# saiprasadbarke/robustmvd

Measured on AMD Instinct MI355X. Metric: depth-maps/sec at 768x1152x4srcx256planes; warp+aggregate HBM GB/s vs roofline, higher is better.
Workload: dtype f32; 1 GPU; mvsnet (Path B) forward 768x1152, 4 source views, 256 planes, batch 1 per step (BASELINE.json configs[2]); the regulariser's two layers with 32 input channels (conv0, conv4): every fp32 operand as two range-scaled fp16 terms on fp16 MFMA, fp32 accumulation (at least as close to a float64 convolution as the fp32 matrix instruction over 1e-42..1e30: tests/test_hip_f16.py), the other nine layers and ; parallelism=1 independent replica(s), frames round-robin, no collectives

## Files before the change

robustmvd_amd/csrc/deconv3d_split.hip:

```cpp
#include "mvd_common.h"
#include "split_operand.h"
#include <stdlib.h>

#ifndef DS_TWO_PHASE
#define DS_TWO_PHASE 0
#endif

namespace mvd {

typedef _Float16 dsh8 __attribute__((ext_vector_type(8)));
typedef float dsf4 __attribute__((ext_vector_type(4)));
typedef unsigned int dsu4 __attribute__((ext_vector_type(4)));

constexpr int DS_TH = 4, DS_ROWS = DS_TH + 1;

template <int CIN, int MT>
struct DSGeom {
    static constexpr bool PAIR = CIN == 16;
    static constexpr int TW = 16 * MT, COLS = TW + 1;
    static constexpr int NG = CIN / 8;
    static constexpr int KS = PAIR ? 1 : CIN / 32;
    static constexpr int PIX = 2 * DS_ROWS * COLS;
    static constexpr int GS = (PIX * 16 + 255) / 256 * 256;
    static constexpr int TERM = NG * GS;
    static constexpr int LDS = 2 * TERM;
    static constexpr int ITEMS = PIX * NG, NIT = (ITEMS + 255) / 256;
    static constexpr int NCLS = PAIR ? 4 : 8;
};
static constexpr int ds_nfrag(int cin) { return cin == 16 ? 9 : 27 * (cin / 32); }
static constexpr size_t DS_FRAG_BYTES = 2 * 64 * 16;

__global__ void deconv_split_pack_kernel(const float* __restrict__ w, const float* __restrict__ eun, _Float16* __restrict__ packed, int Cin,
                                         int Cout, int nfrag, long long total) {
    const long long e = (long long)blockIdx.x * 256 + threadIdx.x;
    if (e >= total) return;
    const int j = (int)(e & 7), lane = (int)((e >> 3) & 63), term = (int)((e >> 9) & 1);
    const int f = (int)((e >> 10) % nfrag), nt = (int)((e >> 10) / nfrag);
    const int row = lane & 15, k = 8 * (lane >> 4) + j;
    int cout, cin, tap;
    if (Cin == 16) {
        const int pw = row >> 3, s = k >> 4;
        const int kw = s == 0 ? (pw ? 2 : 1) : (pw ? 0 : -1);
        cout = row & 7; cin = k & 15;
        tap = kw >= 0 ? f * 3 + kw : -1;
    } else {
        const int ks = f % (Cin / 32);
        cout = nt * 16 + row; cin = 32 * ks + k;
        tap = f / (Cin / 32);
    }
    const float v = tap >= 0 ? w[((size_t)cin * Cout + cout) * 27 + tap] / eun[nt * 16 + row] : 0.f;
    _Float16 hi, lo;
    split_weight(v, 1.0f, hi, lo);
    packed[e] = term == 0 ? hi : lo;
}

struct DSParams {
    const float* x;
    const float* xamax;
    const char* wpk;
    const float* scale;
    const float* shift;
    const float* skip;
    float* y;
    float* yamax;
    int B, Di, hi, wi, Cout, relu;
    int tiles_w, tiles_h, ncb;
};

template <int CIN, int NT, int MT, bool YAMAX>
__global__ void __launch_bounds__(256) deconv3d_split_kernel(DSParams p) {
    const float amax_seen = absmax_seen(YAMAX ? p.yamax : nullptr);
    using G = DSGeom<CIN, MT>;
    constexpr bool PAIR = G::PAIR;
    constexpr int COLS = G::COLS, NG = G::NG, KS = G::KS, GS = G::GS, TERM = G::TERM, NCLS = G::NCLS, NFRAG = ds_nfrag(CIN);
    static_assert(!PAIR || NT == 1, "the pair form has one row tile");
    extern __shared__ __attribute__((aligned(16))) char dslab[];

    const int tid = threadIdx.x;
    const int lane = tid & 63, wave = tid >> 6;
    const int vox = lane & 15, q = lane >> 4;
    int bx = blockIdx.x;
    const int cb = bx % p.ncb; bx /= p.ncb;
    const int tw = bx % p.tiles_w; bx /= p.tiles_w;
    const int th = bx % p.tiles_h; bx /= p.tiles_h;
    const int zd = bx % p.Di;
    const int b = bx / p.Di;
    const int r0 = th * DS_TH, c0 = tw * G::TW;

    float xsc, xsc_inv;
    split_xscale(p.xamax, xsc, xsc_inv);

    constexpr int NKW = PAIR ? 1 : 3;
    const char* __restrict__ wl = p.wpk + (size_t)cb * NT * NFRAG * DS_FRAG_BYTES + lane * 16;
    auto load_a = [&](int step, dsh8 (&dst)[NKW][KS][NT][2]) {
#pragma unroll
        for (int kw = 0; kw < NKW; ++kw)
#pragma unroll
            for (int ks = 0; ks < KS; ++ks)
#pragma unroll
                for (int n = 0; n < NT; ++n)
#pragma unroll
                    for (int t = 0; t < 2; ++t)
                        dst[kw][ks][n][t] = *reinterpret_cast<const dsh8*>(
                            wl + ((size_t)n * NFRAG + (step * NKW + kw) * KS + ks) * DS_FRAG_BYTES + t * 1024);
    };
    constexpr bool AHEAD = 2 * NKW * KS * NT * 2 * 4 <= 112;
    dsh8 af[NKW][KS][NT][2];
    if constexpr (AHEAD) load_a(0, af);

    float emul[NT][4], emul2[NT][4], esc[NT][4], esh[NT][4];
    {
        const float* __restrict__ eun = reinterpret_cast<const float*>(p.wpk + (size_t)p.ncb * NT * NFRAG * DS_FRAG_BYTES);
#pragma unroll
        for (int n = 0; n < NT; ++n)
#pragma unroll
            for (int k = 0; k < 4; ++k) {
                const int row = (cb * NT + n) * 16 + q * 4 + k;
                const int ch = PAIR ? (row & 7) : row;
                const int se = (int)((__float_as_uint(eun[row]) >> 23) & 0xffu) + (int)((__float_as_uint(xsc_inv) >> 23) & 0xffu) - 254;
                emul[n][k] = __uint_as_float((unsigned)(127 + (se >> 1)) << 23);
                emul2[n][k] = __uint_as_float((unsigned)(127 + se - (se >> 1)) << 23);
                esc[n][k] = p.scale[ch];
                esh[n][k] = p.shift[ch];
            }
    }

    {
        constexpr int NIT = G::NIT, C4 = CIN / 4;
        const float4* __restrict__ x4 = reinterpret_cast<const float4*>(p.x) + (size_t)b * p.Di * p.hi * p.wi * C4;
        float4 pf[NIT][2];
        bool ok[NIT];
#pragma unroll
        for (int i = 0; i < NIT; ++i) {
            const int e = tid + 256 * i;
            const int g = e % NG, pix = e / NG;
            const int col = pix % COLS, r = pix / COLS;
            const int pl = r / DS_ROWS, row = r - pl * DS_ROWS;
            const int plane = zd + pl, gr = r0 + row, gc = c0 + col;
            ok[i] = e < G::ITEMS && plane < p.Di && gr < p.hi && gc < p.wi;
            const size_t o = ok[i] ? (((size_t)plane * p.hi + gr) * p.wi + gc) * C4 + 2 * g : 0;
            pf[i][0] = x4[o];
            pf[i][1] = x4[o + 1];
        }
#pragma unroll
        for (int i = 0; i < NIT; ++i) {
            const int e = tid + 256 * i;
            const int g = e % NG, pix = e / NG;
            unsigned h[4], l[4];
            split2(xsc, pf[i][0].x, pf[i][0].y, h[0], l[0]);
            split2(xsc, pf[i][0].z, pf[i][0].w, h[1], l[1]);
            split2(xsc, pf[i][1].x, pf[i][1].y, h[2], l[2]);
            split2(xsc, pf[i][1].z, pf[i][1].w, h[3], l[3]);
            dsu4 hv = {h[0], h[1], h[2], h[3]}, lv = {l[0], l[1], l[2], l[3]};
            if (!ok[i]) { hv = dsu4{0, 0, 0, 0}; lv = dsu4{0, 0, 0, 0}; }
            if (e < G::ITEMS) {
                *reinterpret_cast<dsu4*>(dslab + g * GS + pix * 16) = hv;
                *reinterpret_cast<dsu4*>(dslab + TERM + g * GS + pix * 16) = lv;
            }
        }
    }
    __syncthreads();

    dsf4 acc[NCLS][MT][NT];
#pragma unroll
    for (int c = 0; c < NCLS; ++c)
#pragma unroll
        for (int m = 0; m < MT; ++m)
#pragma unroll
            for (int n = 0; n < NT; ++n) acc[c][m][n] = dsf4{0.f, 0.f, 0.f, 0.f};

    const char* __restrict__ lbase = dslab + (PAIR ? (q & 1) * GS + (q >> 1) * 16 : q * GS) + (wave * COLS + vox) * 16;

#pragma unroll
    for (int step = 0; step < 9; ++step) {
        const int kd = step / 3, kh = step % 3;
        dsh8 af_next[NKW][KS][NT][2];
        if constexpr (AHEAD) {
            if (step + 1 < 9) load_a(step + 1, af_next);
        } else {
            load_a(step, af);
        }
        const int rowpix = ((kd == 0 ? DS_ROWS : 0) + (kh == 0)) * COLS;
#pragma unroll
        for (int kw = 0; kw < NKW; ++kw) {
            const int cls = PAIR ? (((kd != 1) << 1) | (kh != 1)) : (((kd != 1) << 2) | ((kh != 1) << 1) | (kw != 1));
            const int colpix = PAIR ? 0 : (kw == 0);
#pragma unroll
            for (int ks = 0; ks < KS; ++ks) {
                dsh8 xh[MT], xl[MT];
#pragma unroll
                for (int m = 0; m < MT; ++m) {
                    const char* a = lbase + ks * 4 * GS + (rowpix + colpix + m * 16) * 16;
                    xh[m] = *reinterpret_cast<const dsh8*>(a);
                    xl[m] = *reinterpret_cast<const dsh8*>(a + TERM);
                }
#pragma unroll
                for (int m = 0; m < MT; ++m)
#pragma unroll
                    for (int n = 0; n < NT; ++n) {
                        acc[cls][m][n] = __builtin_amdgcn_mfma_f32_16x16x32_f16(af[kw][ks][n][0], xh[m], acc[cls][m][n], 0, 0, 0);
                        acc[cls][m][n] = __builtin_amdgcn_mfma_f32_16x16x32_f16(af[kw][ks][n][1], xh[m], acc[cls][m][n], 0, 0, 0);
                        acc[cls][m][n] = __builtin_amdgcn_mfma_f32_16x16x32_f16(af[kw][ks][n][0], xl[m], acc[cls][m][n], 0, 0, 0);
                    }
            }
        }
        if constexpr (AHEAD) {
            if (step + 1 < 9) {
#pragma unroll
                for (int kw = 0; kw < NKW; ++kw)
#pragma unroll
                    for (int ks = 0; ks < KS; ++ks)
#pragma unroll
                        for (int n = 0; n < NT; ++n) {
                            af[kw][ks][n][0] = af_next[kw][ks][n][0];
                            af[kw][ks][n][1] = af_next[kw][ks][n][1];
                        }
            }
        }
    }

    const int arow = r0 + wave;
    const bool row_ok = arow < p.hi;
    auto offset = [&](int c, int m, int n) {
        const int pd = PAIR ? c >> 1 : c >> 2, ph = PAIR ? c & 1 : (c >> 1) & 1, pw = PAIR ? q >> 1 : c & 1;
        const size_t row_base = (((size_t)b * 2 * p.Di + 2 * zd + pd) * 2 * p.hi + 2 * arow + ph) * 2 * p.wi;
        const int cbase = PAIR ? 4 * (q & 1) : (cb * NT + n) * 16 + q * 4;
        return (row_base + 2 * (c0 + m * 16 + vox) + pw) * p.Cout + cbase;
    };
    auto finish = [&](int c, int m, int n, size_t o) {
        float4 sk = make_float4(0.f, 0.f, 0.f, 0.f);
        if (p.skip) sk = *reinterpret_cast<const float4*>(p.skip + o);
        float r[4];
#pragma unroll
        for (int k = 0; k < 4; ++k) {
            float val = fmaf(acc[c][m][n][k] * emul[n][k] * emul2[n][k], esc[n][k], esh[n][k]);
            if (p.relu) val = fmaxf(val, 0.f);
            r[k] = val;
        }
        return dsf4{r[0] + sk.x, r[1] + sk.y, r[2] + sk.z, r[3] + sk.w};
    };
    if constexpr (!(YAMAX || DS_TWO_PHASE)) {
        if (row_ok) {
#pragma unroll
            for (int c = 0; c < NCLS; ++c)
#pragma unroll
                for (int m = 0; m < MT; ++m) {
                    if (c0 + m * 16 + vox >= p.wi) continue;
#pragma unroll
                    for (int n = 0; n < NT; ++n) {
                        const size_t o = offset(c, m, n);
                        *reinterpret_cast<dsf4*>(p.y + o) = finish(c, m, n, o);
                    }
                }
        }
    } else {
        [[maybe_unused]] float amax = 0.f;
        if (row_ok) {
#pragma unroll
            for (int c = 0; c < NCLS; ++c)
#pragma unroll
                for (int m = 0; m < MT; ++m) {
                    if (c0 + m * 16 + vox >= p.wi) continue;
#pragma unroll
                    for (int n = 0; n < NT; ++n) {
                        const dsf4 out = finish(c, m, n, offset(c, m, n));
                        acc[c][m][n] = out;
                        if constexpr (YAMAX)
                            amax = fmaxf(fmaxf(amax, fmaxf(finite_abs_or_zero(out[0]), finite_abs_or_zero(out[1]))),
                                         fmaxf(finite_abs_or_zero(out[2]), finite_abs_or_zero(out[3])));
                    }
                }
        }
        if constexpr (YAMAX) {
            const float m = workgroup_max(amax, reinterpret_cast<float*>(dslab + G::LDS), tid);
            if (tid == 0) {
                if (m > amax_seen) atomicMax(reinterpret_cast<unsigned*>(p.yamax), __float_as_uint(m));
            }
        }
        if (row_ok) {
#pragma unroll
            for (int c = 0; c < NCLS; ++c)
#pragma unroll
                for (int m = 0; m < MT; ++m) {
                    if (c0 + m * 16 + vox >= p.wi) continue;
#pragma unroll
                    for (int n = 0; n < NT; ++n) *reinterpret_cast<dsf4*>(p.y + offset(c, m, n)) = acc[c][m][n];
                }
        }
    }
}

template <int CIN, int NT, int MT, bool YAMAX>
static int ds_launch_v(DSParams p, hipStream_t st) {
    using G = DSGeom<CIN, MT>;
    static_assert(G::LDS <= 64 * 1024, "slab exceeds the default LDS limit");
    p.tiles_h = (p.hi + DS_TH - 1) / DS_TH;
    p.tiles_w = (p.wi + G::TW - 1) / G::TW;
    p.ncb = G::PAIR ? 1 : p.Cout / (16 * NT);
    const long long nblk = (long long)p.ncb * p.tiles_w * p.tiles_h * p.Di * p.B;
    MVD_REQUIRE(nblk <= 0x7fffffffLL, "deconv3d_split: %lld workgroups exceed the grid limit", nblk);
    hipLaunchKernelGGL((deconv3d_split_kernel<CIN, NT, MT, YAMAX>), dim3((unsigned)nblk), dim3(256), G::LDS + 16, st, p);
    return launch_status("deconv3d_split");
}
template <int CIN, int NT, int MT>
static int ds_launch(const DSParams& p, hipStream_t st) {
    return p.yamax ? ds_launch_v<CIN, NT, MT, true>(p, st) : ds_launch_v<CIN, NT, MT, false>(p, st);
}

}

static bool ds_shape_ok(int Cin, int Cout) {
    return ((Cin == 64 || Cin == 32) && Cout >= 16 && Cout <= 64 && Cout % 16 == 0) || (Cin == 16 && Cout == 8);
}
static int ds_row_tiles(int Cin, int Cout) { return Cin == 16 ? 1 : Cout / 16; }
static size_t ds_frag_bytes(int Cin, int Cout) { return (size_t)ds_row_tiles(Cin, Cout) * mvd::ds_nfrag(Cin) * mvd::DS_FRAG_BYTES; }

extern "C" {

size_t mvd_deconv3d_split_packed_weight_bytes(int Cin, int Cout) {
    return ds_shape_ok(Cin, Cout) ? ds_frag_bytes(Cin, Cout) + (size_t)ds_row_tiles(Cin, Cout) * 16 * sizeof(float) : 0;
}

int mvd_pack_deconv3d_weights_split(const float* w, int Cin, int Cout, void* packed, mvd_stream_t stream) {
    MVD_REQUIRE(w && packed, "pack_deconv3d_weights_split: NULL argument");
    MVD_REQUIRE(ds_shape_ok(Cin, Cout), "pack_deconv3d_weights_split: 32 or 64 input channels with 16, 32, 48 or 64 output channels, or 16 -> 8, are built (got %d -> %d)",
                Cin, Cout);
    float* eun = reinterpret_cast<float*>(static_cast<char*>(packed) + ds_frag_bytes(Cin, Cout));
    const int rows = ds_row_tiles(Cin, Cout) * 16;
    mvd::split_wscale_launch(w, eun, Cin, Cout, 27, true, rows, rows, (hipStream_t)stream);
    const long long total = (long long)(ds_frag_bytes(Cin, Cout) / 2);
    hipLaunchKernelGGL(mvd::deconv_split_pack_kernel, dim3((unsigned)((total + 255) / 256)), dim3(256), 0, (hipStream_t)stream, w, eun,
                       (_Float16*)packed, Cin, Cout, mvd::ds_nfrag(Cin), total);
    return mvd::launch_status("pack_deconv3d_weights_split");
}

int mvd_deconv3d_bn_relu_f32_split(const float* x, const float* x_absmax, const void* packed_w, const float* scale, const float* shift,
                                   const float* skip, float* y, float* y_absmax, int B, int Di, int hi, int wi, int Cin, int Cout, int relu,
                                   mvd_stream_t stream) {
    MVD_REQUIRE(x && x_absmax && packed_w && scale && shift && y, "deconv3d_split: NULL argument");
    MVD_REQUIRE(ds_shape_ok(Cin, Cout), "deconv3d_split: 32 or 64 input channels with 16, 32, 48 or 64 output channels, or 16 -> 8, are built (got %d -> %d)", Cin, Cout);
    MVD_REQUIRE(B > 0 && Di > 0 && hi > 0 && wi > 0, "deconv3d_split: non-positive dimension");
    mvd::DSParams p{};
    p.x = x; p.xamax = x_absmax; p.wpk = (const char*)packed_w; p.scale = scale; p.shift = shift; p.skip = skip; p.y = y; p.yamax = y_absmax;
    p.B = B; p.Di = Di; p.hi = hi; p.wi = wi; p.Cout = Cout; p.relu = relu;
    hipStream_t st = (hipStream_t)stream;
    int cfg = 0;
    if (const char* e = mvd::exp_env("MVD_DS_CFG")) cfg = atoi(e);
    if (Cin == 16) return cfg % 10 == 3 ? mvd::ds_launch<16, 1, 3>(p, st) : mvd::ds_launch<16, 1, 2>(p, st);
    if (Cin == 32) return cfg % 10 == 2 ? mvd::ds_launch<32, 1, 2>(p, st) : mvd::ds_launch<32, 1, 1>(p, st);
    if (cfg / 10 == 2 && Cout % 32 == 0) return mvd::ds_launch<64, 2, 1>(p, st);
    return mvd::ds_launch<64, 1, 1>(p, st);
}
}
```

Before: 340.7 depth-maps/sec.

## Add persistent deconv3d split kernel with prefetched slabs and rolling weight lookahead

Adds a persistent-grid variant of the split-fp16 transposed 3D convolution in which each workgroup loops over tiles. While computing the current tile it prefetches the next tile's input slab and skip values into registers and streams the per-step weight fragments LA steps ahead. For the 16-channel pair form, all weights stay resident. It is enabled by default for the 64-, 32- and 16-input-channel default configurations, and aims to hide global-memory latency and launch/tail overhead. The cost is much higher register pressure, with launch bounds limiting waves per SIMD, and a grid sized to two workgroups per CU equivalent, which may reduce occupancy.

```diff
diff --git a/robustmvd_amd/csrc/deconv3d_split.hip b/robustmvd_amd/csrc/deconv3d_split.hip
--- a/robustmvd_amd/csrc/deconv3d_split.hip
+++ b/robustmvd_amd/csrc/deconv3d_split.hip
@@ -4,6 +4,9 @@
 
 #ifndef DS_TWO_PHASE
 #define DS_TWO_PHASE 0
+#endif
+#ifndef DS_STAGE_PIXMAJOR
+#define DS_STAGE_PIXMAJOR 0
 #endif
 
 namespace mvd {
@@ -65,6 +68,7 @@
     float* yamax;
     int B, Di, hi, wi, Cout, relu;
     int tiles_w, tiles_h, ncb;
+    int tiles;
 };
 
 template <int CIN, int NT, int MT, bool YAMAX>
@@ -290,7 +294,282 @@
     }
 }
 
-template <int CIN, int NT, int MT, bool YAMAX>
+template <int CIN, int NT, int MT, bool YAMAX, int LA, int WAVES, bool SKIP_EARLY, bool PIXMAJOR>
+__global__ void __launch_bounds__(256, WAVES) deconv3d_split_persist_kernel(DSParams p) {
+    const float amax_seen = absmax_seen(YAMAX ? p.yamax : nullptr);
+    using G = DSGeom<CIN, MT>;
+    constexpr bool PAIR = G::PAIR;
+    constexpr int COLS = G::COLS, NG = G::NG, KS = G::KS, GS = G::GS, TERM = G::TERM, NCLS = G::NCLS, NFRAG = ds_nfrag(CIN);
+    constexpr int NIT = G::NIT, C4 = CIN / 4, NKW = PAIR ? 1 : 3;
+    static_assert(!PAIR || NT == 1, "the pair form has one row tile");
+    static_assert(LA >= 1 && LA <= 9 && (LA < 9 || PAIR), "resident weights: the pair form (one channel block) only");
+    static_assert(NIT <= 32, "one bit per staging item");
+    extern __shared__ __attribute__((aligned(16))) char dslab[];
+
+    const int tid = threadIdx.x;
+    const int lane = tid & 63, wave = __builtin_amdgcn_readfirstlane(tid >> 6);
+    const int vox = lane & 15, q = lane >> 4;
+    int t = blockIdx.x;
+    if (t >= p.tiles) return;
+
+    float xsc, xsc_inv;
+    split_xscale(p.xamax, xsc, xsc_inv);
+
+    struct Tile { int cb, b, zd, r0, c0; };
+    auto tile_of = [&](int bx) {
+        Tile tl;
+        tl.cb = bx % p.ncb; bx /= p.ncb;
+        tl.c0 = (bx % p.tiles_w) * G::TW; bx /= p.tiles_w;
+        tl.r0 = (bx % p.tiles_h) * DS_TH; bx /= p.tiles_h;
+        tl.zd = bx % p.Di;
+        tl.b = bx / p.Di;
+        return tl;
+    };
+
+    struct Item { int loff, pl, row, col, g; };
+    auto item_of = [&](int i, int tz) {
+        const int e = tid + tz + 256 * i;
+        const int g = PIXMAJOR ? e / G::PIX : e % NG, pix = PIXMAJOR ? e % G::PIX : e / NG;
+        const int col = pix % COLS, r = pix / COLS;
+        const int pl = r / DS_ROWS;
+        return Item{e < G::ITEMS ? g * GS + pix * 16 : -1, pl, r - pl * DS_ROWS, col, g};
+    };
+    float4 pf[NIT][2];
+    unsigned okm = 0;
+    auto prefetch = [&](const Tile& tl) {
+        const float4* __restrict__ x4 = reinterpret_cast<const float4*>(p.x) + (size_t)tl.b * p.Di * p.hi * p.wi * C4;
+        okm = 0;
+        int tz = 0;
+        asm volatile("" : "+v"(tz));
+#pragma unroll
+        for (int i = 0; i < NIT; ++i) {
+            const Item it = item_of(i, tz);
+            const int plane = tl.zd + it.pl, gr = tl.r0 + it.row, gc = tl.c0 + it.col;
+            const bool ok = it.loff >= 0 && plane < p.Di && gr < p.hi && gc < p.wi;
+            const size_t o = ok ? (((size_t)plane * p.hi + gr) * p.wi + gc) * C4 + 2 * it.g : 0;
+            pf[i][0] = x4[o];
+            pf[i][1] = x4[o + 1];
+            okm |= (ok ? 1u : 0u) << i;
+        }
+    };
+
+    dsh8 w[9][NKW][KS][NT][2];
+    auto load_w = [&](int cb, int step) {
+        const char* __restrict__ wl = p.wpk + (size_t)cb * NT * NFRAG * DS_FRAG_BYTES + lane * 16;
+#pragma unroll
+        for (int kw = 0; kw < NKW; ++kw)
+#pragma unroll
+            for (int ks = 0; ks < KS; ++ks)
+#pragma unroll
+                for (int n = 0; n < NT; ++n)
+#pragma unroll
+                    for (int tm = 0; tm < 2; ++tm)
+                        w[step][kw][ks][n][tm] = *reinterpret_cast<const dsh8*>(
+                            wl + ((size_t)n * NFRAG + (step * NKW + kw) * KS + ks) * DS_FRAG_BYTES + tm * 1024);
+    };
+
+    float emul[NT][4], emul2[NT][4], esc[NT][4], esh[NT][4];
+    auto load_consts = [&](int cb) {
+        const float* __restrict__ eun = reinterpret_cast<const float*>(p.wpk + (size_t)p.ncb * NT * NFRAG * DS_FRAG_BYTES);
+#pragma unroll
+        for (int n = 0; n < NT; ++n)
+#pragma unroll
+            for (int k = 0; k < 4; ++k) {
+                const int row = (cb * NT + n) * 16 + q * 4 + k;
+                const int ch = PAIR ? (row & 7) : row;
+                const int se = (int)((__float_as_uint(eun[row]) >> 23) & 0xffu) + (int)((__float_as_uint(xsc_inv) >> 23) & 0xffu) - 254;
+                emul[n][k] = __uint_as_float((unsigned)(127 + (se >> 1)) << 23);
+                emul2[n][k] = __uint_as_float((unsigned)(127 + se - (se >> 1)) << 23);
+                esc[n][k] = p.scale[ch];
+                esh[n][k] = p.shift[ch];
+            }
+    };
+
+    const char* __restrict__ lbase = dslab + (PAIR ? (q & 1) * GS + (q >> 1) * 16 : q * GS) + (wave * COLS + vox) * 16;
+    const float* __restrict__ skp = p.skip ? p.skip : p.y;
+
+    Tile tl = tile_of(t);
+    load_consts(tl.cb);
+    int cb_have = tl.cb;
+    prefetch(tl);
+#pragma unroll
+    for (int s = 0; s < LA; ++s) load_w(tl.cb, s);
+    [[maybe_unused]] float amax = 0.f;
+
+    for (;;) {
+        const int tn = t + (int)gridDim.x;
+        const bool more = tn < p.tiles;
+        Tile tnext;
+        if (tl.cb != cb_have) {
+            load_consts(tl.cb);
+            cb_have = tl.cb;
+        }
+
+        const int arow = tl.r0 + wave;
+        const bool row_ok = arow < p.hi;
+        const size_t obase = ((((size_t)tl.b * 2 * p.Di + 2 * tl.zd) * 2 * p.hi + 2 * arow) * 2 * p.wi + 2 * tl.c0) * p.Cout + (PAIR ? 0 : tl.cb * NT * 16);
+        auto delta = [&](int c, int m, int n) {
+            const int pd = PAIR ? c >> 1 : c >> 2, ph = PAIR ? c & 1 : (c >> 1) & 1, pw = PAIR ? 0 : c & 1;
+            return ((pd * 2 * p.hi + ph) * 2 * p.wi + 32 * m + pw) * p.Cout + 16 * n;
+        };
+        const int lane_off = (2 * vox + (PAIR ? q >> 1 : 0)) * p.Cout + (PAIR ? 4 * (q & 1) : q * 4);
+        bool has[MT];
+#pragma unroll
+        for (int m = 0; m < MT; ++m) has[m] = row_ok && tl.c0 + m * 16 + vox < p.wi;
+
+        __builtin_amdgcn_sched_barrier(0);
+        __syncthreads();
+        int tz = 0;
+        asm volatile("" : "+v"(tz));
+#pragma unroll
+        for (int i = 0; i < NIT; ++i) {
+            const int lo = item_of(i, tz).loff;
+            if (lo < 0) continue;
+            unsigned h[4], l[4];
+            split2(xsc, pf[i][0].x, pf[i][0].y, h[0], l[0]);
+            split2(xsc, pf[i][0].z, pf[i][0].w, h[1], l[1]);
+            split2(xsc, pf[i][1].x, pf[i][1].y, h[2], l[2]);
+            split2(xsc, pf[i][1].z, pf[i][1].w, h[3], l[3]);
+            dsu4 hv = {h[0], h[1], h[2], h[3]}, lv = {l[0], l[1], l[2], l[3]};
+            if (!((okm >> i) & 1u)) { hv = dsu4{0, 0, 0, 0}; lv = dsu4{0, 0, 0, 0}; }
+            *reinterpret_cast<dsu4*>(dslab + lo) = hv;
+            *reinterpret_cast<dsu4*>(dslab + TERM + lo) = lv;
+        }
+        __builtin_amdgcn_sched_barrier(0);
+
+        float4 sk[NCLS][MT][NT];
+        auto request_skip = [&]() {
+#pragma unroll
+            for (int c = 0; c < NCLS; ++c)
+#pragma unroll
+                for (int m = 0; m < MT; ++m)
+#pragma unroll
+                    for (int n = 0; n < NT; ++n) sk[c][m][n] = *reinterpret_cast<const float4*>(
+                            skp + (row_ok ? obase : 0) + (unsigned)(row_ok && tl.c0 + m * 16 < p.wi ? delta(c, m, n) + (has[m] ? lane_off : 0) : 0));
+        };
+        auto request_skip_and_slab = [&]() {
+            if constexpr (SKIP_EARLY) request_skip();
+            tnext = tile_of(more ? tn : t);
+            prefetch(tnext);
+        };
+        if constexpr (LA == 9) {
+            request_skip_and_slab();
+            __builtin_amdgcn_sched_barrier(0);
+        }
+        __syncthreads();
+
+        dsf4 acc[NCLS][MT][NT];
+#pragma unroll
+        for (int c = 0; c < NCLS; ++c)
+#pragma unroll
+            for (int m = 0; m < MT; ++m)
+#pragma unroll
+                for (int n = 0; n < NT; ++n) acc[c][m][n] = dsf4{0.f, 0.f, 0.f, 0.f};
+
+#pragma unroll
+        for (int step = 0; step < 9; ++step) {
+            const int kd = step / 3, kh = step % 3;
+            if constexpr (LA < 9) {
+                if (step + LA < 9) load_w(tl.cb, step + LA);
+                else load_w(tnext.cb, step + LA - 9);
+                if (step == 8 - LA) request_skip_and_slab();
+                __builtin_amdgcn_sched_barrier(0);
+            }
+            const int rowpix = ((kd == 0 ? DS_ROWS : 0) + (kh == 0)) * COLS;
+#pragma unroll
+            for (int kw = 0; kw < NKW; ++kw) {
+                const int cls = PAIR ? (((kd != 1) << 1) | (kh != 1)) : (((kd != 1) << 2) | ((kh != 1) << 1) | (kw != 1));
+                const int colpix = PAIR ? 0 : (kw == 0);
+#pragma unroll
+                for (int ks = 0; ks < KS; ++ks) {
+                    dsh8 xh[MT], xl[MT];
+#pragma unroll
+                    for (int m = 0; m < MT; ++m) {
+                        const char* a = lbase + ks * 4 * GS + (rowpix + colpix + m * 16) * 16;
+                        xh[m] = *reinterpret_cast<const dsh8*>(a);
+                        xl[m] = *reinterpret_cast<const dsh8*>(a + TERM);
+                    }
+#pragma unroll
+                    for (int m = 0; m < MT; ++m)
+#pragma unroll
+                        for (int n = 0; n < NT; ++n) {
+                            acc[cls][m][n] = __builtin_amdgcn_mfma_f32_16x16x32_f16(w[step][kw][ks][n][0], xh[m], acc[cls][m][n], 0, 0, 0);
+                            acc[cls][m][n] = __builtin_amdgcn_mfma_f32_16x16x32_f16(w[step][kw][ks][n][1], xh[m], acc[cls][m][n], 0, 0, 0);
+                            acc[cls][m][n] = __builtin_amdgcn_mfma_f32_16x16x32_f16(w[step][kw][ks][n][0], xl[m], acc[cls][m][n], 0, 0, 0);
+                        }
+                }
+            }
+        }
+        __builtin_amdgcn_sched_barrier(0);
+        if constexpr (!SKIP_EARLY) request_skip();
+
+#pragma unroll
+        for (int c = 0; c < NCLS; ++c)
+#pragma unroll
+            for (int m = 0; m < MT; ++m)
+#pragma unroll
+                for (int n = 0; n < NT; ++n) {
+                    float r[4];
+#pragma unroll
+                    for (int k = 0; k < 4; ++k) {
+                        float val = fmaf(acc[c][m][n][k] * emul[n][k] * emul2[n][k], esc[n][k], esh[n][k]);
+                        if (p.relu) val = fmaxf(val, 0.f);
+                        r[k] = val;
+                    }
+                    const float4 s4 = p.skip ? sk[c][m][n] : make_float4(0.f, 0.f, 0.f, 0.f);
+                    const dsf4 out = {r[0] + s4.x, r[1] + s4.y, r[2] + s4.z, r[3] + s4.w};
+                    if (has[m]) {
+                        if constexpr (YAMAX)
+                            amax = fmaxf(fmaxf(amax, fmaxf(finite_abs_or_zero(out[0]), finite_abs_or_zero(out[1]))),
+                                         fmaxf(finite_abs_or_zero(out[2]), finite_abs_or_zero(out[3])));
+                        *reinterpret_cast<dsf4*>(p.y + obase + (unsigned)(delta(c, m, n) + lane_off)) = out;
+                    }
+                }
+        if (!more) break;
+        t = tn;
+        tl = tnext;
+    }
+    if constexpr (YAMAX) {
+        const float m = workgroup_max(amax, reinterpret_cast<float*>(dslab + G::LDS), tid);
+        if (tid == 0) {
+            if (m > amax_seen) atomicMax(reinterpret_cast<unsigned*>(p.yamax), __float_as_uint(m));
+        }
+    }
+}
+
+enum { DS_CONV7 = 0, DS_CONV9 = 1, DS_CONV11 = 2 };
+constexpr int DS_PERSIST_WGS[3] = {2, 2, 2};
+template <int CIN> struct DSPersist;
+template <> struct DSPersist<64> { static constexpr int LAYER = DS_CONV7, LA = 1, WAVES = 2, ALT_LA = 1, ALT_WAVES = 2; static constexpr bool SKIP_EARLY = false, ALT_SKIP_EARLY = false; };
+template <> struct DSPersist<32> { static constexpr int LAYER = DS_CONV9, LA = 2, WAVES = 2, ALT_LA = 1, ALT_WAVES = 2; static constexpr bool SKIP_EARLY = true, ALT_SKIP_EARLY = true; };
+template <> struct DSPersist<16> { static constexpr int LAYER = DS_CONV11, LA = 9, WAVES = 2, ALT_LA = 2, ALT_WAVES = 3; static constexpr bool SKIP_EARLY = true, ALT_SKIP_EARLY = false; };
+#ifdef MVD_EXPERIMENTS
+constexpr bool DS_EXP = true;
+#else
+constexpr bool DS_EXP = false;
+#endif
+static long long ds_persist_grid(int layer, long long tiles, int ncb, long long plane_floats) {
+    if (tiles > 0x3fffffffLL || plane_floats > (1LL << 28)) return 0;
+    const int wgs = DS_PERSIST_WGS[layer];
+    if (const char* e = exp_env("MVD_DS_PERSIST")) {
+        const long long v = atoll(e);
+        if (v <= 0) return 0;
+        if (v > 1) return v < tiles ? v : tiles;
+    }
+    if (wgs == 0) return 0;
+    const long long grid = (256LL * wgs + ncb - 1) / ncb * ncb;
+    return grid < tiles ? grid : tiles;
+}
+
+template <int CIN, int NT, int MT, bool YAMAX, int LA, int WAVES, bool SKIP_EARLY>
+static int ds_launch_persist(const DSParams& p, long long grid, hipStream_t st) {
+    using G = DSGeom<CIN, MT>;
+    hipLaunchKernelGGL((deconv3d_split_persist_kernel<CIN, NT, MT, YAMAX, LA, WAVES, SKIP_EARLY, DS_STAGE_PIXMAJOR != 0>), dim3((unsigned)grid), dim3(256),
+                       G::LDS + 16, st, p);
+    return launch_status("deconv3d_split: persistent");
+}
+
+template <int CIN, int NT, int MT, bool YAMAX, bool PERSIST>
 static int ds_launch_v(DSParams p, hipStream_t st) {
     using G = DSGeom<CIN, MT>;
     static_assert(G::LDS <= 64 * 1024, "slab exceeds the default LDS limit");
@@ -299,12 +578,24 @@
     p.ncb = G::PAIR ? 1 : p.Cout / (16 * NT);
     const long long nblk = (long long)p.ncb * p.tiles_w * p.tiles_h * p.Di * p.B;
     MVD_REQUIRE(nblk <= 0x7fffffffLL, "deconv3d_split: %lld workgroups exceed the grid limit", nblk);
+    if constexpr (PERSIST && (DS_EXP || DS_PERSIST_WGS[DSPersist<CIN>::LAYER] > 0)) {
+        using P = DSPersist<CIN>;
+        if (const long long grid = ds_persist_grid(P::LAYER, nblk, p.ncb, (2LL * p.hi + 2) * 2 * p.wi * p.Cout)) {
+            p.tiles = (int)nblk;
+#ifdef MVD_EXPERIMENTS
+            if (const char* e = exp_env("MVD_DS_LA")) {
+                if (P::ALT_LA != P::LA && atoi(e) == P::ALT_LA) return ds_launch_persist<CIN, NT, MT, YAMAX, P::ALT_LA, P::ALT_WAVES, P::ALT_SKIP_EARLY>(p, grid, st);
+            }
+#endif
+            return ds_launch_persist<CIN, NT, MT, YAMAX, P::LA, P::WAVES, P::SKIP_EARLY>(p, grid, st);
+        }
+    }
     hipLaunchKernelGGL((deconv3d_split_kernel<CIN, NT, MT, YAMAX>), dim3((unsigned)nblk), dim3(256), G::LDS + 16, st, p);
     return launch_status("deconv3d_split");
 }
-template <int CIN, int NT, int MT>
+template <int CIN, int NT, int MT, bool PERSIST = false>
 static int ds_launch(const DSParams& p, hipStream_t st) {
-    return p.yamax ? ds_launch_v<CIN, NT, MT, true>(p, st) : ds_launch_v<CIN, NT, MT, false>(p, st);
+    return p.yamax ? ds_launch_v<CIN, NT, MT, true, PERSIST>(p, st) : ds_launch_v<CIN, NT, MT, false, PERSIST>(p, st);
 }
 
 }
@@ -346,9 +637,9 @@
     hipStream_t st = (hipStream_t)stream;
     int cfg = 0;
     if (const char* e = mvd::exp_env("MVD_DS_CFG")) cfg = atoi(e);
-    if (Cin == 16) return cfg % 10 == 3 ? mvd::ds_launch<16, 1, 3>(p, st) : mvd::ds_launch<16, 1, 2>(p, st);
-    if (Cin == 32) return cfg % 10 == 2 ? mvd::ds_launch<32, 1, 2>(p, st) : mvd::ds_launch<32, 1, 1>(p, st);
+    if (Cin == 16) return cfg % 10 == 3 ? mvd::ds_launch<16, 1, 3>(p, st) : mvd::ds_launch<16, 1, 2, true>(p, st);
+    if (Cin == 32) return cfg % 10 == 2 ? mvd::ds_launch<32, 1, 2>(p, st) : mvd::ds_launch<32, 1, 1, true>(p, st);
     if (cfg / 10 == 2 && Cout % 32 == 0) return mvd::ds_launch<64, 2, 1>(p, st);
-    return mvd::ds_launch<64, 1, 1>(p, st);
-}
-}
+    return mvd::ds_launch<64, 1, 1, true>(p, st);
+}
+}
```

Measured after the change: 348.6 depth-maps/sec (median of 6 runs). 2.3% higher.
